# GAP-LAB-CUHK-SZ/RfDNet

Hardware: AMD Instinct MI355X
Metric: scenes/sec end-to-end reconstruction (ScanNet, 64^3 MISE) (higher is better)
Workload: dtype f32 (point ops, MLPs); f16x3 split MFMA with f32 accumulate (decoder, fp32-class)

## Files before the change

include/rfd_occ.h:

```cpp
#ifndef RFD_OCC_H
#define RFD_OCC_H

#include <stddef.h>

#ifdef __cplusplus
extern "C" {
#endif

#define RFD_OCC_HIDDEN 256
#define RFD_OCC_BLOCKS 5
#define RFD_OCC_TILE 128
#define RFD_OCC_TABLE_ROWS 23

#define RFD_OCC_MODE_F16X3 3
#define RFD_OCC_MODE_F16X1 1

size_t rfd_occ_packed_bytes(void);

int rfd_occ_pack_weights(const float *fc0_w, const float *fc1_w,
                         const int *kw0, int kw1, void *packed, void *stream);

int rfd_occ_decode(int n_tiles, const float *pts, const int *tile_prop,
                   const int *tile_src, const void *packed, const float *fc_p_w, const float *table,
                   const float *fc_out_w, float fc_out_b, float *logits,
                   int mode, void *stream);

int rfd_make_grid_points(int n, float lo, float hi, float scale, float *pts,
                         int n_padded, void *stream);

size_t rfd_mise_vstate_elems(int res0, int depth);
int rfd_mise_init(int K, int res0, int depth, unsigned char *pstate,
                  unsigned char *vstate, void *stream);
int rfd_mise_count(int K, int res0, int depth, const unsigned char *pstate,
                   int *counts, void *stream);
int rfd_mise_collect(int K, int res0, int depth, const unsigned char *pstate,
                     const int *offsets, int *cursors, float box_size,
                     float *pts, int *lin, void *stream);
int rfd_mise_scatter(int n_tiles, int res0, int depth, const int *tile_prop,
                     const int *tile_src, const int *lin, const float *logits,
                     float *values, unsigned char *pstate, void *stream);
int rfd_mise_subdivide(int K, int res0, int depth, double threshold,
                       const float *values, unsigned char *pstate,
                       unsigned char *vstate, void *stream);
int rfd_mise_subdivide_active(int K, int res0, int depth, double threshold, const float *values,
                              unsigned char *pstate, unsigned char *vstate, const int *evaluated,
                              void *stream);
size_t rfd_mise_dirty_elems(int res0, int depth);
int rfd_mise_subdivide_dirty(int K, int res0, int depth, double threshold, const float *values,
                             unsigned char *pstate, unsigned char *vstate, const int *evaluated, long long n_slots,
                             const int *lin, const int *tile_prop, unsigned char *dirty_cur,
                             unsigned char *dirty_next, int use_dirty, void *stream);
int rfd_mise_to_dense(int K, int res0, int depth, float *values,
                      unsigned char *pstate, void *stream);

int rfd_mc_blocks(int n);
int rfd_mc_classify(int K, int n, float pad_value, double iso, const float *grids,
                    unsigned char *code, int *vsum, int *tsum, void *stream);
int rfd_mc_emit_affine(int K, int n, float pad_value, double iso, const float *grids,
                       const unsigned char *code, const int *vblock, const int *tblock,
                       int *vbase, double *verts, int *tris, double va, double vc, void *stream);

int rfd_points_in_boxes(int b, int K, int n, int point_stride, const float *pts,
                        const double *boxes, int *counts, void *stream);
int rfd_nms3d(int b, int K, double iou_thr, int old_type, int use_cls, const double *aabb,
              const int *order, const int *cls, const unsigned char *valid,
              unsigned char *keep, void *stream);

int rfd_occ_pack_weights_w8(const float *fc0_w, const float *fc1_w, const int *kw0, int kw1,
                            void *packed, void *stream);
int rfd_occ_decode_w8(int n_tiles, const float *pts, const int *tile_prop, const int *tile_src,
                      const void *packed, const float *fc_p_w, const float *table,
                      const float *fc_out_w, float fc_out_b, float *logits, int mode, void *stream);
int rfd_occ_decode_scatter_w8(int n_tiles, const float *pts, const int *tile_prop, const int *tile_src,
                              const void *packed, const float *fc_p_w, const float *table,
                              const float *fc_out_w, float fc_out_b, const int *lin, float *values,
                              unsigned char *pstate, long long n_per, int mode, void *stream);

int rfd_occ_chunk_range(int k, int n_tiles, int n_workgroups, int *begin, int *end);
int rfd_occ_set_launch_shape(int static_partition, int cus, int chunk_cap);
int rfd_occ_set_tail_tiles(int n_tiles);
int rfd_occ_chunk_range_capped(int k, int n_tiles, int n_workgroups, int max_chunk, int *begin, int *end,
                               int *n_chunks);

int rfd_occ_normals_w8(int n_groups, const double *verts, const int *vend, const int *gprefix, int K,
                       const void *packed_fwd, const void *packed_bwd, const int *kw, const float *fc_p_w,
                       const float *table, const float *fc_out_w, float *normals, float *grad, int mode,
                       void *stream);

int rfd_refine_sample(int F, int K, const float *verts, const int *faces, const int *fend, const int *vend,
                      const int *tprefix, const float *eps, double *qd, float *qt, void *stream);
int rfd_refine_face_backward(int F, int K, const float *verts, const int *faces, const int *fend, const int *vend,
                             const int *tprefix, const float *eps, const float *logits, const float *grad, float tau,
                             double *cg, void *stream);
int rfd_refine_vertex_step(int V, const int *rowptr, const int *col, int n_corners, const double *cg, float *verts,
                           float *sq, float *gout, void *stream);
int rfd_refine_dirichlet(int n, unsigned long long seed, int step, float *out, void *stream);

size_t rfd_gemm_packed_bytes(int N, int K);
int rfd_gemm_pack_w(int N, int K, int sw, const float *W, void *packed, void *stream);
int rfd_gemm_f16x3(int M, int N, int K, const float *A, int lda, const void *packed_w,
                   float *C, int ldc, const float *bias, const float *gbias,
                   int rows_per_group, const float *R, int ldr, int relu_in, int relu_out,
                   int sa, int sw, float *pool_max, int pool_signed, void *stream);

// ... 37 lines not shown
```

rfdnet_amd/_lib.py:

```python
import ctypes as C
import os

_HERE = os.path.dirname(os.path.abspath(__file__))
LIB_PATH = os.environ.get("RFD_HIP_LIB") or os.path.join(_HERE, "lib", "librfd_hip.so")

_f = C.c_void_p
_i = C.c_int
_fl = C.c_float
_sz = C.c_size_t
_d = C.c_double

OPTIONAL = "optional"
ABI = {
    "furthest_point_sampling_kernel_wrapper": (_i, [_i, _i, _i, _f, _f, _f, _f]),
    "gather_points_kernel_wrapper": (_i, [_i, _i, _i, _i, _f, _f, _f, _f]),
    "gather_points_grad_kernel_wrapper": (_i, [_i, _i, _i, _i, _f, _f, _f, _f]),
    "query_ball_point_kernel_wrapper": (_i, [_i, _i, _i, _fl, _i, _f, _f, _f, _f]),
    "group_points_kernel_wrapper": (_i, [_i, _i, _i, _i, _i, _f, _f, _f, _f]),
    "group_points_grad_kernel_wrapper": (_i, [_i, _i, _i, _i, _i, _f, _f, _f, _f]),
    "three_nn_kernel_wrapper": (_i, [_i, _i, _i, _f, _f, _f, _f, _f]),
    "three_interpolate_kernel_wrapper": (_i, [_i, _i, _i, _i, _f, _f, _f, _f, _f]),
    "three_interpolate_grad_kernel_wrapper": (_i, [_i, _i, _i, _i, _f, _f, _f, _f, _f]),
    "rfd_group_concat": (_i, [_i, _i, _i, _i, _i, _fl, _i, _i, _f, _f, _f, _f, _f, _f, _f]),
    "rfd_furthest_point_sampling_gather": (_i, [_i, _i, _i, _f, _f, _f, _f, _f]),
    "rfd_chamfer_forward": (_i, [_i, _i, _f, _i, _f, _f, _f, _f, _f, _f]),
    "rfd_chamfer_backward": (_i, [_i, _i, _f, _i, _f, _f, _f, _f, _f, _f, _f, _f]),
    "rfd_sa_fused": (_i, [_i, _i, _i, _i, _i, _fl, _i, _f, _f, _f, _f, _i, _i, _i, _f, _f, _f, _f, _f, _f, _f, _f]),
    "rfd_occ_pack_weights": (_i, [_f, _f, C.POINTER(C.c_int), _i, _f, _f]),
    "rfd_occ_decode": (_i, [_i, _f, _f, _f, _f, _f, _f, _f, _fl, _f, _i, _f]),
    "rfd_occ_pack_weights_w8": (_i, [_f, _f, C.POINTER(C.c_int), _i, _f, _f]),
    "rfd_occ_decode_w8": (_i, [_i, _f, _f, _f, _f, _f, _f, _f, _fl, _f, _i, _f]),
    "rfd_occ_decode_scatter_w8": (_i, [_i, _f, _f, _f, _f, _f, _f, _f, _fl, _f, _f, _f, C.c_longlong, _i, _f]),
    "rfd_occ_chunk_range": (_i, [_i, _i, _i, C.POINTER(C.c_int), C.POINTER(C.c_int)]),
    "rfd_occ_chunk_range_capped": (_i, [_i, _i, _i, _i, C.POINTER(C.c_int), C.POINTER(C.c_int), C.POINTER(C.c_int)]),
    "rfd_occ_set_launch_shape": (_i, [_i, _i, _i]),
    "rfd_occ_set_tail_tiles": (_i, [_i]),
    "rfd_occ_normals_w8": (_i, [_i, _f, _f, _f, _i, _f, _f, C.POINTER(C.c_int), _f, _f, _f, _f, _f, _i, _f]),
    "rfd_refine_sample": (_i, [_i, _i, _f, _f, _f, _f, _f, _f, _f, _f, _f]),
    "rfd_refine_face_backward": (_i, [_i, _i, _f, _f, _f, _f, _f, _f, _f, _f, _fl, _f, _f]),
    "rfd_refine_vertex_step": (_i, [_i, _f, _f, _i, _f, _f, _f, _f, _f]),
    "rfd_refine_dirichlet": (_i, [_i, C.c_ulonglong, _i, _f, _f]),
    "rfd_fps_set_timeout_ms": (_i, [_i]),
    "rfd_fps_set_geometry": (_i, [_i]),
    "rfd_test_hold_cus": (_i, [_i, _f, _i, _f], OPTIONAL),
    "rfd_fps_test_phantom_units": (_i, [_i], OPTIONAL),
    "rfd_make_grid_points": (_i, [_i, _fl, _fl, _fl, _f, _i, _f]),
    "rfd_mise_init": (_i, [_i, _i, _i, _f, _f, _f]),
    "rfd_mise_count": (_i, [_i, _i, _i, _f, _f, _f]),
    "rfd_mise_collect": (_i, [_i, _i, _i, _f, _f, _f, _fl, _f, _f, _f]),
    "rfd_mise_scatter": (_i, [_i, _i, _i, _f, _f, _f, _f, _f, _f, _f]),
    "rfd_mise_subdivide": (_i, [_i, _i, _i, C.c_double, _f, _f, _f, _f]),
    "rfd_mise_subdivide_active": (_i, [_i, _i, _i, C.c_double, _f, _f, _f, _f, _f]),
    "rfd_mise_subdivide_dirty": (_i, [_i, _i, _i, C.c_double, _f, _f, _f, _f, C.c_longlong, _f, _f, _f, _f, _i, _f]),
    "rfd_mise_to_dense": (_i, [_i, _i, _i, _f, _f, _f]),
    "rfd_points_in_boxes": (_i, [_i, _i, _i, _i, _f, _f, _f, _f]),
    "rfd_nms3d": (_i, [_i, _i, C.c_double, _i, _i, _f, _f, _f, _f, _f, _f]),
    "rfd_gemm_pack_w": (_i, [_i, _i, _i, _f, _f, _f]),
    "rfd_gemm_f16x3": (_i, [_i, _i, _i, _f, _i, _f, _f, _i, _f, _f, _i, _f, _i, _i, _i, _i, _i, _f, _i, _f]),
    "rfd_mc_classify": (_i, [_i, _i, _fl, C.c_double, _f, _f, _f, _f, _f]),
    "rfd_mc_emit_affine": (_i, [_i, _i, _fl, C.c_double, _f, _f, _f, _f, _f, _f, _f, C.c_double, C.c_double, _f]),
    "rfd_mc_blocks": (_i, [_i]),
    "rfd_occ_fold_rows": (_i, [_i, _i, _i, _f, _f, _f, _f, _f, _f, _f, _i, _f, _f]),
    "rfd_rows3_rotate_z": (_i, [_i, _i, _f, _f, _f, _f]),
    "rfd_rows3_affine": (_i, [_i, _i, _f, _f, _f, _f]),
    "rfd_mlp_cols": (_i, [_i, _i, _i, _f, _f, _f, _f, _f, _f, _f]),
    "rfd_three_interpolate_cat": (_i, [_i, _i, _i, _i, _i, _f, _f, _f, _f, _f, _f]),
    "rfd_chain_pack_n": (_i, [_i, _i, _f, _f, _f, _i, _i, _i, _f, _f]),
    "rfd_chain_pool_n": (_i, [_i, _i, _i, _i, _i, _f, _i, _f, _f, _f, _f, _f, _i, _i, _i, _i, _i, _f, _f]),
    "rfd_head_pack": (_i, [_f, _f, _f, _i, _i, _i, _f, _f]),
    "rfd_head_scores": (_i, [_i, _i, _f, _i, _f, _f, _f, _f, _f, _f, _i, _i, _i, _i, _i, _f, _f]),
    "rfd_pos_embed": (_i, [_i, _i, _i, _f, _i, _f, _f, _i, _f, _f, _i, _f, _i, _i, _f]),
    "rfd_pos_embed_frag": (_i, [_i, _i, _i, _f, _i, _f, _f, _i, _f, _f, _i, _f, C.c_long, _i, _f]),
    "rfd_rows_to_frag": (_i, [_i, _i, _f, _i, _i, _i, _f, C.c_long, _f]),
    "rfd_frag_to_rows": (_i, [_i, _i, _f, C.c_long, _i, _f, _i, _f]),
    "rfd_gemm_f16x3_frag": (_i, [_i, _i, _i, _f, C.c_long, _f, _f, C.c_long, _f, _f, _i, _i, _i, _i, _f, _i, _f]),
    "rfd_box3d_iou": (_i, [_i, _i, _i, _f, _f, _f, _f, _f]),
    "rfd_ap_match": (_i, [_i, _i, _i, _i, _i, _f, _f, _f, _f, _f, _f, _f, _f]),
    "rfd_latent_prep": (_i, [_i, _i, _f, _f, _f, _f, _f, _f]),
    "rfd_latent_stage": (_i, [_i, _i, _i, _f, _f, _f, _f, _f, _f, _f, _f, _f]),
    "rfd_latent_head": (_i, [_i, _i, _f, _f, _f, _f, _f, _f, _f, _f, _f]),
    "rfd_bce_logits_rowsum": (_i, [_i, _i, _f, _i, _f, _i, _f, _f]),
    "rfd_voxel_iou": (_i, [_i, _i, _f, _i, _fl, _f, _f, _f, _f]),
    "rfd_vote_loss_partial": (_i, [_i, _i, _i, _i, _f, _f, _f, _f, _f, _f, _f]),
    "rfd_proposal_loss_partial": (_i, [_i, _i, _i, _i, _i, _i, _f, _f, _f, _f, _f, _f, _f, _f, C.POINTER(C.c_int), _f, _i, _f, _f,
                                       _f, _f, _f, _f, _f, _f, _f, _f, _i, _f, _f]),
    "rfd_detection_loss_finish": (_i, [_i, _i, _i, _f, _f, _f]),
    "rfd_mask_loss_partial": (_i, [_i, _i, _f, _f, _i, _f, _f, _f, _f]),
    "rfd_mask_loss_finish": (_i, [_i, _i, _fl, _f, _f, _f]),
    "rfd_fit_pose_run": (_i, [_i, _i, _i, _i, _i, _i, C.c_double, C.c_double, _f, _f, _f, _f, _f, _f, _f, _f, _f, _f, _f, _f,
                              _f, _f]),
    "rfd_raster_project": (_i, [_i, _i, _i, _f, _f, C.POINTER(C.c_double), C.c_double, _f, _f, _f, _f]),
    "rfd_raster_triangles": (_i, [_i, _i, _i, _i, _i, _i, _f, _f, _f, _f, _f, _f]),
    "rfd_raster_shade": (_i, [_i, _i, _i, _i, _i, _f, _f, _f, _f, _f, C.POINTER(C.c_double), _f, _f, _f, _f, _f]),
    "rfd_decimate_vertex_keys": (_i, [_i, _i, _i, _i, _f, _f, _f, _f, _f, _f]),
    "rfd_decimate_face_remap": (_i, [_i, _i, _i, _f, _f, _f, _f, _f, _f, _f, _f, _f]),
    "rfd_decimate_parity": (_i, [_i, _i, _i, _f, _f, _f, _f, _f, _f, _f]),
    "rfd_decimate_cell_solve": (_i, [_i, _i, _i, _i, _i, _f, _f, _f, _f, _f, _f, _f, _f, _f, C.c_double, _f, _f]),
    "rfd_decimate_compact_faces": (_i, [_i, _i, _f, _f, _f, _f, _f, _f, _f, _f]),
    "rfd_simplify_init": (_i, [_i, _i, _i, _i, _f, _f, _f, _f, _f, _f, _f, _f, _f]),
    "rfd_simplify_quadrics": (_i, [_i, _i, _f, _f, _f, _f, _f, _f]),
    "rfd_simplify_edges": (_i, [_i, _i, _f, _f, _f, _f, _f, _f, _f, _f, _f, _f]),
    "rfd_simplify_edge_costs": (_i, [_i, _i, _i, _f, _f, _f, _f, _f, _f, _f, _f, _f, _f, _f, _f, _f, _f, _f, _f]),
    "rfd_simplify_vertex_min": (_i, [_i, _i, _i, _f, _f, _f, _f, _f, _f, _f]),
    "rfd_simplify_select": (_i, [_i, _i, _f, _f, _f, _f, _f, _f, _f]),
    "rfd_simplify_apply": (_i, [_i, _i, _f, _f, _f, _f, _f, _f, _f, _f, _f, _f, _f]),
    "rfd_simplify_compact_faces": (_i, [_i, _i, _i, _f, _f, _f, _f, _f, _f, _f, _f, _f, _f, _f]),
# ... 247 lines not shown
```

rfdnet_amd/csrc/mise.hip:

```cpp
#include "common.h"
#include "../../include/rfd_occ.h"

namespace {

__host__ __device__ inline size_t cube(size_t n) { return n * n * n; }

__host__ __device__ inline size_t vstate_offset(int res0, int l) {
  size_t o = 0;
  for (int i = 0; i < l; ++i) o += cube((size_t)res0 << i);
  return o;
}

__global__ void grid_points_kernel(int n, float lo, float hi, float scale,
                                   float *__restrict__ pts, int n_padded) {
  const int e = blockIdx.x * blockDim.x + threadIdx.x;
  if (e >= n_padded) return;
  const int total = n * n * n;
  float x = 0.f, y = 0.f, z = 0.f;
  if (e < total) {
    const int k = e % n, j = (e / n) % n, i = e / (n * n);
    const float step = n > 1 ? (hi - lo) / (float)(n - 1) : 0.f;
    const int half = n / 2;
    auto ax = [&](int q) { return q < half ? lo + step * (float)q : hi - step * (float)(n - 1 - q); };
    x = scale * ax(i);
// ... 111 lines not shown
__global__ __launch_bounds__(256) void mise_collect_kernel(
    int R1, size_t total, size_t n_per, int K, const unsigned char *__restrict__ pstate,
    const int *__restrict__ offsets, int *__restrict__ cursors, float box_size,
    float *__restrict__ pts, int *__restrict__ lin) {
  const size_t chunk = (size_t)blockIdx.x * blockDim.x + threadIdx.x;
  const int lane = threadIdx.x & 63;
  unsigned m = 0, lo = 0xffffu;
  int k0 = -1;
  size_t e0 = 0;
  if (chunk * 16 < total) {
    const Chunk c = load_chunk(pstate, total, n_per, chunk);
    m = unknown_mask16(c);
    lo = c.split >= 16 ? 0xffffu : ((1u << c.split) - 1u);
    k0 = c.k0;
    e0 = c.e0;
  }
  const int c0 = __popc(m & lo), c1 = __popc(m & ~lo);
  if (!__any(c0 | c1)) return;
  int base0 = 0, base1 = 0;
  const int kf = __shfl(k0, 0);
  if (__all((k0 == kf || (c0 | c1) == 0) && c1 == 0)) {
    int incl = c0;
#pragma unroll
    for (int off = 1; off < 64; off <<= 1) {
      const int o = __shfl_up(incl, off);
      if (lane >= off) incl += o;
    }
    const int tot = __shfl(incl, 63);
    int wb = 0;
    if (lane == 0) wb = atomicAdd(cursors + kf, tot);
    wb = __shfl(wb, 0);
    base0 = wb + incl - c0;
  } else {
    if (c0) base0 = atomicAdd(cursors + k0, c0);
    if (c1 && k0 + 1 < K) base1 = atomicAdd(cursors + k0 + 1, c1);
  }
  const float res = (float)(R1 - 1);
  unsigned mm = m;
  while (mm) {
    const int j = __ffs(mm) - 1;
    mm &= mm - 1;
    const bool second = !((lo >> j) & 1u);
    const int k = second ? k0 + 1 : k0;
    if (k >= K) break;
    const unsigned e = (unsigned)(second ? (e0 + j - n_per) : (e0 + j));
    const int slot = offsets[k] + (second ? base1++ : base0++);
    const unsigned row = e / (unsigned)R1;
    const int kz = (int)(e - row * (unsigned)R1), ix = (int)(row / (unsigned)R1),
              jy = (int)(row - (unsigned)ix * (unsigned)R1);
    pts[(size_t)slot * 3 + 0] = box_size * ((float)ix / res - 0.5f);
    pts[(size_t)slot * 3 + 1] = box_size * ((float)jy / res - 0.5f);
    pts[(size_t)slot * 3 + 2] = box_size * ((float)kz / res - 0.5f);
    lin[slot] = (int)e;
  }
}

__global__ void mise_scatter_kernel(size_t n_per, const int *__restrict__ tile_prop,
                                    const int *__restrict__ tile_src,
                                    const int *__restrict__ lin,
                                    const float *__restrict__ logits,
                                    float *__restrict__ values,
                                    unsigned char *__restrict__ pstate) {
  const int tile = blockIdx.x;
  const int k = tile_prop[tile];
  if (k < 0) return;
  const size_t slot = (size_t)tile * RFD_OCC_TILE + threadIdx.x;
  const int l = lin[tile_src ? (size_t)tile_src[tile] * RFD_OCC_TILE + threadIdx.x : slot];
  if (l < 0) return;
  values[(size_t)k * n_per + l] = logits[slot];
  pstate[(size_t)k * n_per + l] = 2;
}

constexpr int SUB_TJ = 8, SUB_TK = 32;

__host__ __device__ inline int sub_tiles_k(int nl) { return (nl + SUB_TK - 1) / SUB_TK; }
__host__ __device__ inline int sub_tiles_j(int nl) { return (nl + SUB_TJ - 1) / SUB_TJ; }
__host__ __device__ inline size_t dirty_offset(int res0, int l) {
  size_t o = 0;
  for (int i = 0; i < l; ++i) {
    const int nl = res0 << i;
    o += (size_t)sub_tiles_k(nl) * sub_tiles_j(nl) * nl;
  }
  return o;
}
__device__ inline size_t dirty_tile(int nl, int vi, int vj, int vk) {
  return ((size_t)vi * sub_tiles_j(nl) + vj / SUB_TJ) * sub_tiles_k(nl) + vk / SUB_TK;
}
__device__ inline void mark_children(unsigned char *dirty_next, int res0, int l, int nl, int vi, int vj, int vk) {
  unsigned char *d = dirty_next + dirty_offset(res0, l + 1);
  d[dirty_tile(2 * nl, 2 * vi, 2 * vj, 2 * vk)] = 1;
  d[dirty_tile(2 * nl, 2 * vi + 1, 2 * vj, 2 * vk)] = 1;
}

__global__ void mise_mark_dirty_kernel(size_t n_slots, int R1, int res0, int depth, const int *__restrict__ lin,
                                       const int *__restrict__ tile_prop, size_t d_per,
                                       unsigned char *__restrict__ dirty) {
  const size_t i = (size_t)blockIdx.x * blockDim.x + threadIdx.x;
  if (i >= n_slots) return;
  const int p = lin[i];
  if (p < 0) return;
  const int kp = tile_prop[i / RFD_OCC_TILE];
  if (kp < 0) return;
  const int c[3] = {p / (R1 * R1), (p / R1) % R1, p % R1};
  unsigned char *dk = dirty + (size_t)kp * d_per;
  for (int l = 0; l < depth; ++l) {
    const int s = 1 << (depth - l), nl = res0 << l;
// ... 114 lines not shown
#pragma unroll
      for (int i = 0; i < 16; ++i) {
        const int rel = rel0 + i;
        if (rel < 0 || rel >= plane) continue;
        unsigned char f = 0;
        if (rel < run && ((w[i >> 2] >> (8 * (i & 3))) & 0xffu) == 2u) {
          const double v = (double)vals[base + rel];
          f = 4 | (v >= thr ? 1 : 0) | (v <= thr ? 2 : 0);
        }
        flags[a * plane + rel] = f;
      }
    }
  } else {
    for (int t = threadIdx.x; t < (s + 1) * PJ * PK; t += SUB_TJ * SUB_TK) {
      const int c = t % PK, b = (t / PK) % PJ, a = t / (PK * PJ);
      unsigned char f = 0;
      if (y0 + b < R1 && z0 + c < R1) {
        const size_t p = ((size_t)(x0 + a) * R1 + (y0 + b)) * R1 + (z0 + c);
        if (ps[p] == 2) {
          const double v = (double)vals[p];
          f = 4 | (v >= thr ? 1 : 0) | (v <= thr ? 2 : 0);
        }
      }
      flags[t] = f;
    }
  }
  __syncthreads();
  if (!leaf) return;
  unsigned any = 0;
  for (int a = 0; a <= s; ++a)
    for (int b = 0; b <= s; ++b)
      for (int c = 0; c <= s; ++c)
        any |= flags[(a * PJ + tj * s + b) * PK + tk * s + c];
  if ((any & 3) != 3) return;
  vs[e] = 2;
  if (l + 1 < depth) {
    unsigned char *vc = vstate + (size_t)kp * v_per + vstate_offset(res0, l + 1);
    const int nc = nl * 2;
    for (int a = 0; a < 2; ++a)
      for (int b = 0; b < 2; ++b)
        for (int c = 0; c < 2; ++c)
          vc[((size_t)(2 * vi + a) * nc + (2 * vj + b)) * nc + (2 * vk + c)] = 1;
    if (dirty_next) mark_children(dirty_next + (size_t)kp * d_per, res0, l, nl, vi, vj, vk);
  }
  const int h = s >> 1;
  for (int a = 0; a < 3; ++a)
    for (int b = 0; b < 3; ++b)
      for (int c = 0; c < 3; ++c) {
        const size_t p = ((size_t)(x0 + a * h) * R1 + (y0 + tj * s + b * h)) * R1 + (z0 + tk * s + c * h);
        if (ps[p] == 0) ps[p] = 1;
      }
}

__global__ void mise_fill_kernel(int R1, int axis, size_t n_per, float *__restrict__ values,
                                 unsigned char *__restrict__ pstate) {
  const int line = blockIdx.x * blockDim.x + threadIdx.x;
  if (line >= R1 * R1) return;
  const int kp = blockIdx.y;
  const int u = line / R1, v = line % R1;
  size_t stride, start;
  if (axis == 0) { stride = (size_t)R1 * R1; start = (size_t)u * R1 + v; }
  else if (axis == 1) { stride = R1; start = (size_t)u * R1 * R1 + v; }
  else { stride = 1; start = ((size_t)u * R1 + v) * R1; }
  float *vals = values + (size_t)kp * n_per;
  unsigned char *ps = pstate + (size_t)kp * n_per;
  bool prev_valid = false;
  float prev = 0.f;
  for (int q0 = 0; q0 < R1; q0 += 8) {
    float v[8];
    unsigned char st[8];
#pragma unroll
    for (int u = 0; u < 8; ++u) {
      const bool in = q0 + u < R1;
      const size_t p = start + (size_t)(q0 + u) * stride;
      st[u] = in ? ps[p] : 0;
      v[u] = in ? vals[p] : 0.f;
    }
#pragma unroll
    for (int u = 0; u < 8; ++u) {
      if (q0 + u >= R1) break;
      const size_t p = start + (size_t)(q0 + u) * stride;
      const bool valid = st[u] >= 2;
      if (!valid && prev_valid) {
        vals[p] = prev;
        ps[p] = 3;
      }
      prev = valid ? v[u] : prev;
      prev_valid = valid || prev_valid;
    }
  }
}

__global__ __launch_bounds__(256) void mise_fill_yz_kernel(int R1, size_t n_per,
                                                           float *__restrict__ values,
                                                           const unsigned char *__restrict__ pstate) {
  extern __shared__ float plane_v[];
  const int n2 = R1 * R1;
  unsigned char *plane_s = reinterpret_cast<unsigned char *>(plane_v + n2);
  const size_t base = (size_t)blockIdx.y * n_per + (size_t)blockIdx.x * n2;
  for (int t = threadIdx.x; t < n2; t += 256) {
    plane_v[t] = values[base + t];
    plane_s[t] = pstate[base + t];
  }
  __syncthreads();
  for (int axis = 1; axis <= 2; ++axis) {
    if ((int)threadIdx.x < R1) {
// ... 59 lines not shown
  RFD_CHECK_LAUNCH();
  return 0;
}

RFD_API size_t rfd_mise_vstate_elems(int res0, int depth) {
  const size_t v = vstate_offset(res0, depth);
  return v ? v : 1;
}

RFD_API int rfd_mise_init(int K, int res0, int depth, unsigned char *pstate,
                          unsigned char *vstate, void *stream) {
  if (K <= 0) return 0;
  const int R1 = (res0 << depth) + 1;
  const size_t n_per = cube((size_t)R1);
  hipStream_t s = (hipStream_t)stream;
  RFD_CHECK(hipMemsetAsync(pstate, 0, n_per * (size_t)K, s));
  const int L = res0 + 1;
  hipLaunchKernelGGL(mise_init_points_kernel, dim3((unsigned)((L * L * L + 255) / 256), K), dim3(256),
                     0, s, R1, 1 << depth, L, n_per, pstate);
  RFD_CHECK_LAUNCH();
  const size_t v_per = rfd_mise_vstate_elems(res0, depth);
  hipLaunchKernelGGL(mise_init_voxels_kernel, dim3((unsigned)((v_per + 255) / 256), K), dim3(256),
                     0, s, depth > 0 ? cube((size_t)res0) : 0, v_per, vstate);
  RFD_CHECK_LAUNCH();
  return 0;
}

RFD_API int rfd_mise_count(int K, int res0, int depth, const unsigned char *pstate,
                           int *counts, void *stream) {
  if (K <= 0) return 0;
  const int R1 = (res0 << depth) + 1;
  const size_t n_per = cube((size_t)R1);
  hipStream_t s = (hipStream_t)stream;
  RFD_CHECK(hipMemsetAsync(counts, 0, sizeof(int) * K, s));
  hipLaunchKernelGGL(mise_count_kernel, dim3(COUNT_PARTS, K), dim3(256), 0, s, n_per, pstate, counts);
  RFD_CHECK_LAUNCH();
  return 0;
}

RFD_API int rfd_mise_collect(int K, int res0, int depth, const unsigned char *pstate,
                             const int *offsets, int *cursors, float box_size,
                             float *pts, int *lin, void *stream) {
  if (K <= 0) return 0;
  const int R1 = (res0 << depth) + 1;
  const size_t n_per = cube((size_t)R1);
  const size_t total = n_per * (size_t)K, chunks = (total + 15) / 16;
  hipLaunchKernelGGL(mise_collect_kernel, dim3((unsigned)((chunks + 255) / 256)), dim3(256), 0,
                     (hipStream_t)stream, R1, total, n_per, K, pstate, offsets, cursors, box_size,
                     pts, lin);
  RFD_CHECK_LAUNCH();
  return 0;
}

RFD_API int rfd_mise_scatter(int n_tiles, int res0, int depth, const int *tile_prop,
                             const int *tile_src, const int *lin, const float *logits,
                             float *values, unsigned char *pstate, void *stream) {
  if (n_tiles <= 0) return 0;
  const int R1 = (res0 << depth) + 1;
  hipLaunchKernelGGL(mise_scatter_kernel, dim3(n_tiles), dim3(RFD_OCC_TILE), 0,
                     (hipStream_t)stream, cube((size_t)R1), tile_prop, tile_src, lin, logits, values,
                     pstate);
  RFD_CHECK_LAUNCH();
  return 0;
}

static int mise_subdivide(int K, int res0, int depth, double threshold, const float *values,
                          unsigned char *pstate, unsigned char *vstate, const int *evaluated, void *stream,
                          const unsigned char *dirty_cur = nullptr, unsigned char *dirty_next = nullptr) {
  if (K <= 0 || depth <= 0) return 0;
  const int R1 = (res0 << depth) + 1;
  const size_t n_per = cube((size_t)R1);
  const size_t v_per = rfd_mise_vstate_elems(res0, depth);
  const size_t d_per = dirty_offset(res0, depth);
  for (int l = depth - 1; l >= 0; --l) {
    const size_t nvox = cube((size_t)res0 << l);
    const int sl = 1 << (depth - l), nl = res0 << l;
    if (sl <= 4) {
      const unsigned tiles = (unsigned)(ceil_div(nl, SUB_TK) * ceil_div(nl, SUB_TJ) * nl);
      const size_t lds = (size_t)(sl + 1) * (SUB_TJ * sl + 1) * (SUB_TK * sl + 1);
      hipLaunchKernelGGL(mise_subdivide_lds_kernel, dim3(tiles, K), dim3(SUB_TJ * SUB_TK), lds,
                         (hipStream_t)stream, R1, res0, depth, l, threshold, n_per, v_per,
                         n_per * (size_t)K, values, pstate, vstate, evaluated, d_per, dirty_cur, dirty_next);
      RFD_CHECK_LAUNCH();
      continue;
    }
    hipLaunchKernelGGL(mise_subdivide_kernel, dim3((unsigned)((nvox + 255) / 256), K), dim3(256), 0,
                       (hipStream_t)stream, R1, res0, depth, l, threshold, n_per, v_per, values,
                       pstate, vstate, evaluated, d_per, dirty_next);
    RFD_CHECK_LAUNCH();
  }
  return 0;
}

RFD_API int rfd_mise_subdivide(int K, int res0, int depth, double threshold,
                               const float *values, unsigned char *pstate,
                               unsigned char *vstate, void *stream) {
  return mise_subdivide(K, res0, depth, threshold, values, pstate, vstate, nullptr, stream);
}

RFD_API int rfd_mise_subdivide_active(int K, int res0, int depth, double threshold,
                                      const float *values, unsigned char *pstate,
                                      unsigned char *vstate, const int *evaluated, void *stream) {
  return mise_subdivide(K, res0, depth, threshold, values, pstate, vstate, evaluated, stream);
}

RFD_API size_t rfd_mise_dirty_elems(int res0, int depth) { return dirty_offset(res0, depth); }

RFD_API int rfd_mise_subdivide_dirty(int K, int res0, int depth, double threshold, const float *values,
                                     unsigned char *pstate, unsigned char *vstate, const int *evaluated,
                                     long long n_slots, const int *lin, const int *tile_prop, unsigned char *dirty_cur,
                                     unsigned char *dirty_next, int use_dirty, void *stream) {
  if (K <= 0 || depth <= 0) return 0;
  if (!dirty_cur || !dirty_next || (use_dirty && (!lin || !tile_prop || n_slots < 0))) {
    return rfd_invalid("rfd_mise_subdivide_dirty: dirty maps / query list");
  }
  const int R1 = (res0 << depth) + 1;
  const size_t d_per = dirty_offset(res0, depth);
  if (use_dirty && n_slots > 0) {
    hipLaunchKernelGGL(mise_mark_dirty_kernel, dim3((unsigned)((n_slots + 255) / 256)), dim3(256), 0, (hipStream_t)stream,
                       (size_t)n_slots, R1, res0, depth, lin, tile_prop, d_per, dirty_cur);
    RFD_CHECK_LAUNCH();
  }
  const int rc = mise_subdivide(K, res0, depth, threshold, values, pstate, vstate, evaluated, stream,
                                use_dirty ? dirty_cur : nullptr, dirty_next);
  if (rc) return rc;
  RFD_CHECK(hipMemsetAsync(dirty_cur, 0, (size_t)K * d_per, (hipStream_t)stream));
  return 0;
}

RFD_API int rfd_mise_to_dense(int K, int res0, int depth, float *values,
                              unsigned char *pstate, void *stream) {
  if (K <= 0) return 0;
  const int R1 = (res0 << depth) + 1;
  const size_t n_per = cube((size_t)R1);
  const size_t plane_lds = (size_t)R1 * R1 * 5;
  const bool fused = plane_lds <= 64 * 1024 && R1 <= 256;
  for (int axis = 0; axis < (fused ? 1 : 2); ++axis) {
    hipLaunchKernelGGL(mise_fill_kernel, dim3(ceil_div(R1 * R1, 256), K), dim3(256), 0,
                       (hipStream_t)stream, R1, axis, n_per, values, pstate);
    RFD_CHECK_LAUNCH();
  }
  if (fused)
    hipLaunchKernelGGL(mise_fill_yz_kernel, dim3(R1, K), dim3(256), plane_lds, (hipStream_t)stream,
                       R1, n_per, values, pstate);
  else
    hipLaunchKernelGGL(mise_fill_z_kernel, dim3(ceil_div(R1 * R1, 4), K), dim3(256), 0,
                       (hipStream_t)stream, R1, n_per, values, pstate);
  RFD_CHECK_LAUNCH();
  return 0;
}
```

rfdnet_amd/iscnet/generator.py:

```python
import os

import numpy as np
import torch

from .. import _lib, mesh_batch, ragged
from .occ_decoder import GROUP, MODE_F16X3, TILE, logit_threshold, run_with_range_fallback


class Mesh(object):

    def __init__(self, vertices, faces, vertex_normals=None):
        self.vertices = vertices
        self.faces = faces
        self.vertex_normals = vertex_normals


def draw_dirichlet(face_counts, steps):
    total = int(sum(face_counts))
    out = np.empty((steps, total, 3), dtype=np.float32)
    at = 0
    for n in face_counts:
        for it in range(steps):
            if n:
                out[it, at:at + n] = np.random.dirichlet((0.5, 0.5, 0.5), size=n)
# ... 62 lines not shown
        return self.extract_meshes(grids, fold=fold[0] if self._needs_fold() else None)

    def generate_from_latent(self, z, c=None, device='cuda', **kwargs):
        fold = []
        grids = self._grids(z, c, fold_out=fold)
        return self.extract_meshes(grids, fold=fold[0] if self._needs_fold() else None)[0]

    def eval_points(self, p, z, c=None, device='cuda', **kwargs):
        with torch.no_grad():
            return self.model.decode(p.unsqueeze(0).to(c.device), z, c, **kwargs).logits.squeeze(0)

    def logit_threshold(self):
        return logit_threshold(self.threshold)

    def generate_grids(self, object_features, cls_codes=None, fold_out=None):
        self.model.eval()
        if getattr(self.model, 'use_cls_for_completion', False):
            object_features = torch.cat([object_features, cls_codes], dim=-1)
        K = object_features.size(0)
        z = self.model.get_z_from_prior((K,), sample=self.sample, device=object_features.device)
        return self._grids(z, object_features, fold_out=fold_out)

    @torch.no_grad()
    def _grids(self, z, c, fold_out=None):
        dec = self.model.decoder
        dev = c.device
        K = c.size(0)
        box_size = 1 + self.padding
        table, fc_p_w = dec.fold(z.float(), c.float())
        if fold_out is not None:
            fold_out.append((table, fc_p_w))
        if self.upsampling_steps == 0:
            nx = self.resolution0
            total = nx ** 3
            tiles_per = int(ragged.blocks(total, TILE))
            pts = torch.empty(tiles_per * TILE, 3, dtype=torch.float32, device=dev)
            _lib.call("rfd_make_grid_points", dev, nx, -0.5, 0.5, float(box_size), pts.data_ptr(),
                      tiles_per * TILE)
            tile_prop, tile_src = ragged.uniform_maps(K, tiles_per, dev)
            logits = dec.decode_tiles(pts, tile_prop, table, fc_p_w, tile_src=tile_src)
            self.stats = {'n_queries': K * total, 'rounds': 1, 'per_round': [K * total]}
            return logits.view(K, tiles_per * TILE)[:, :total].reshape(K, nx, nx, nx)
        return self._grids_mise(dec, table, fc_p_w, K, dev, box_size)

    def _grids_mise(self, dec, table, fc_p_w, K, dev, box_size):
        res0, depth = self.resolution0, self.upsampling_steps
        R1 = (res0 << depth) + 1
        n_per = R1 ** 3
        lib = _lib.lib()
        v_per = lib.rfd_mise_vstate_elems(res0, depth)
        values = torch.empty(K, n_per, dtype=torch.float32, device=dev)
        pstate = torch.empty(K, n_per, dtype=torch.uint8, device=dev)
        vstate = torch.empty(K, v_per, dtype=torch.uint8, device=dev)
        counts = torch.empty(K, dtype=torch.int32, device=dev)
        dirty = torch.zeros(2, K, lib.rfd_mise_dirty_elems(res0, depth), dtype=torch.uint8, device=dev)
        _lib.call("rfd_mise_init", dev, K, res0, depth, pstate.data_ptr(), vstate.data_ptr())
        thr = self.logit_threshold()
        n_queries, rounds = 0, 0
        per_round = []
        while True:
            shared = rounds == 0 and self._round0(res0, depth, box_size, K, dev)
            if shared:
                pts, lin, tile_prop, tile_src, total = shared
                n_tiles = tile_prop.numel()
            else:
                _lib.call("rfd_mise_count", dev, K, res0, depth, pstate.data_ptr(), counts.data_ptr())
                cnt = counts.cpu().numpy().astype(np.int64)
                total = int(cnt.sum())
                if total == 0:
                    break
                tiles = ragged.padded_tiles(cnt, TILE)
                n_tiles = int(tiles.prefix[-1])
                tile_prop = ragged.to_int32(tiles.owner, dev)
                tile_src = None
                offsets = ragged.to_int32(tiles.slot[:-1], dev)
                cursors = torch.zeros(K, dtype=torch.int32, device=dev)
                pts = torch.zeros(n_tiles * TILE, 3, dtype=torch.float32, device=dev)
                lin = torch.full((n_tiles * TILE,), -1, dtype=torch.int32, device=dev)
                _lib.call("rfd_mise_collect", dev, K, res0, depth, pstate.data_ptr(), offsets.data_ptr(),
                          cursors.data_ptr(), float(box_size), pts.data_ptr(), lin.data_ptr())
            if self.round_hook is not None:
                self.round_hook(rounds, depth)
            if dec.can_scatter():
                dec.decode_tiles(pts, tile_prop, table, fc_p_w, tile_src=tile_src, scatter=(lin, values, pstate))
            else:
                logits = dec.decode_tiles(pts, tile_prop, table, fc_p_w, tile_src=tile_src)
                _lib.call("rfd_mise_scatter", dev, n_tiles, res0, depth, tile_prop.data_ptr(),
                          _lib.ptr(tile_src), lin.data_ptr(), logits.data_ptr(), values.data_ptr(), pstate.data_ptr())
            sparse = (not shared) and total <= K * self.sparse_round_points
            _lib.call("rfd_mise_subdivide_dirty", dev, K, res0, depth, float(thr), values.data_ptr(),
                      pstate.data_ptr(), vstate.data_ptr(), None if shared else counts.data_ptr(),
                      int(lin.numel()) if sparse else 0, lin.data_ptr() if sparse else None,
                      tile_prop.data_ptr() if sparse else None, dirty[rounds & 1].data_ptr(),
                      dirty[(rounds + 1) & 1].data_ptr(), int(sparse))
            n_queries += total
            per_round.append(total)
            rounds += 1
        _lib.call("rfd_mise_to_dense", dev, K, res0, depth, values.data_ptr(), pstate.data_ptr())
        self.stats = {'n_queries': n_queries, 'rounds': rounds, 'per_round': per_round}
        return values.view(K, R1, R1, R1)

    def _round0(self, res0, depth, box_size, K, dev):
        def build():
            R1 = (res0 << depth) + 1
            ps = torch.empty(1, R1 ** 3, dtype=torch.uint8, device=dev)
            vs = torch.empty(1, _lib.lib().rfd_mise_vstate_elems(res0, depth), dtype=torch.uint8, device=dev)
            cnt = torch.empty(1, dtype=torch.int32, device=dev)
            _lib.call("rfd_mise_init", dev, 1, res0, depth, ps.data_ptr(), vs.data_ptr())
            _lib.call("rfd_mise_count", dev, 1, res0, depth, ps.data_ptr(), cnt.data_ptr())
            n = int(cnt.item())
            tiles_per = int(ragged.blocks(n, TILE))
            pts = torch.zeros(tiles_per * TILE, 3, dtype=torch.float32, device=dev)
            lin = torch.full((tiles_per * TILE,), -1, dtype=torch.int32, device=dev)
            offsets = torch.zeros(1, dtype=torch.int32, device=dev)
            cursors = torch.zeros(1, dtype=torch.int32, device=dev)
            _lib.call("rfd_mise_collect", dev, 1, res0, depth, ps.data_ptr(), offsets.data_ptr(),
                      cursors.data_ptr(), float(box_size), pts.data_ptr(), lin.data_ptr())
            return (pts, lin) + ragged.uniform_maps(K, tiles_per, dev) + (K * n,)
        return self._round0_cache.get((res0, depth, float(box_size), K, str(dev)), build, dev)

    def extract_meshes(self, grids, fold=None):
        from .mcubes import marching_cubes_batch
        thr = self.logit_threshold()
        n = grids.shape[1]
        box_size = 1 + self.padding
        a = box_size / (n - 1)
        v, f, vend, tend = marching_cubes_batch(grids, thr, pad_value=-1e6, return_flat=True,
                                                affine=(a, -1.5 * a - 0.5 * box_size))
        if self.decimate_cells:
            from .decimate import decimate_meshes
            K = len(vend) - 1
            v, f, vend, tend = decimate_meshes(v, f, vend, tend, self.decimate_cells, lo=np.full((K, 3), -box_size / 2),
                                               h=np.full(K, box_size / self.decimate_cells))
        if self.simplify_faces:
            from .simplify import simplify_meshes
            v, f, vend, tend, _ = simplify_meshes(v, f, vend, tend, self.simplify_faces)
        self.last_normals = None
        refine = self.refinement_step > 0
        if refine and fold is None:
            raise ValueError("refinement needs fold = (table, fc_p_w) of the meshes' codes (DecoderCBatchNorm.fold)")
        nrm = None
        if fold is not None and (self.with_normals or not refine):
            nrm = self.last_normals = self.model.decoder.normals(v if v.dtype == torch.float64 else v.double(), vend,
                                                                 fold[0], fold[1])
        if refine:
            v = self.refine_meshes(v, f, vend, tend, fold, self.refinement_step)
        self.last_buffers = (v, f, vend, tend)
# ... 104 lines not shown
```

Baseline: 20.10.

## Fuse MISE round-0 subdivide with counting and pad-aware wave-level collect

Adds a dedicated round-0 subdivide kernel that evaluates the coarse lattice in LDS tiles, marks split voxels and children, and accumulates per-proposal point counts in one pass, so round 1 skips the separate count kernel. Replaces the collect kernel with a wave-compacting version that uses block-level cursor reservation when a block covers one proposal and writes tile padding itself, which removes the zero/fill initialisation of pts and lin. Dirty buffers and counts now share one zeroed allocation. The round-0 path relies on counts being zero at entry and falls back to the generic path when LDS needs exceed 64 KB.

```diff
diff --git a/include/rfd_occ.h b/include/rfd_occ.h
--- a/include/rfd_occ.h
+++ b/include/rfd_occ.h
@@ -50,6 +50,12 @@
                              unsigned char *pstate, unsigned char *vstate, const int *evaluated, long long n_slots,
                              const int *lin, const int *tile_prop, unsigned char *dirty_cur,
                              unsigned char *dirty_next, int use_dirty, void *stream);
+int rfd_mise_subdivide_round0(int K, int res0, int depth, double threshold, const float *values,
+                              unsigned char *pstate, unsigned char *vstate, unsigned char *dirty_next,
+                              int *counts, void *stream);
+int rfd_mise_collect_padded(int K, int res0, int depth, const unsigned char *pstate, const int *counts,
+                            const int *offsets, int *cursors, float box_size, int pad_to, float *pts, int *lin,
+                            void *stream);
 int rfd_mise_to_dense(int K, int res0, int depth, float *values,
                       unsigned char *pstate, void *stream);
 
diff --git a/rfdnet_amd/_lib.py b/rfdnet_amd/_lib.py
--- a/rfdnet_amd/_lib.py
+++ b/rfdnet_amd/_lib.py
@@ -52,6 +52,8 @@
     "rfd_mise_subdivide": (_i, [_i, _i, _i, C.c_double, _f, _f, _f, _f]),
     "rfd_mise_subdivide_active": (_i, [_i, _i, _i, C.c_double, _f, _f, _f, _f, _f]),
     "rfd_mise_subdivide_dirty": (_i, [_i, _i, _i, C.c_double, _f, _f, _f, _f, C.c_longlong, _f, _f, _f, _f, _i, _f]),
+    "rfd_mise_subdivide_round0": (_i, [_i, _i, _i, C.c_double, _f, _f, _f, _f, _f, _f]),
+    "rfd_mise_collect_padded": (_i, [_i, _i, _i, _f, _f, _f, _f, _fl, _i, _f, _f, _f]),
     "rfd_mise_to_dense": (_i, [_i, _i, _i, _f, _f, _f]),
     "rfd_points_in_boxes": (_i, [_i, _i, _i, _i, _f, _f, _f, _f]),
     "rfd_nms3d": (_i, [_i, _i, C.c_double, _i, _i, _f, _f, _f, _f, _f, _f]),
diff --git a/rfdnet_amd/csrc/mise.hip b/rfdnet_amd/csrc/mise.hip
--- a/rfdnet_amd/csrc/mise.hip
+++ b/rfdnet_amd/csrc/mise.hip
@@ -187,6 +187,131 @@
     pts[(size_t)slot * 3 + 1] = box_size * ((float)jy / res - 0.5f);
     pts[(size_t)slot * 3 + 2] = box_size * ((float)kz / res - 0.5f);
     lin[slot] = (int)e;
+  }
+}
+
+constexpr int COL_SEG = 4;
+
+__device__ __forceinline__ unsigned unknown_mask16(const uint4 v) {
+  Chunk c;
+  c.w[0] = v.x; c.w[1] = v.y; c.w[2] = v.z; c.w[3] = v.w;
+  return unknown_mask16(c);
+}
+
+__global__ __launch_bounds__(256) void mise_collect_wave_kernel(
+    int R1, size_t total, size_t n_per, int K, const unsigned char *__restrict__ pstate,
+    const int *__restrict__ counts, const int *__restrict__ offsets, int *__restrict__ cursors, float box_size,
+    int pad_to, float *__restrict__ pts, int *__restrict__ lin) {
+  __shared__ unsigned short rel[4][1024];
+  __shared__ int unit_base[4 * COL_SEG];
+  const int lane = threadIdx.x & 63, wave = threadIdx.x >> 6;
+  const size_t wave_b0 = ((size_t)blockIdx.x * 4 + wave) * (size_t)(COL_SEG * 1024);
+  uint4 v[COL_SEG];
+#pragma unroll
+  for (int q = 0; q < COL_SEG; ++q) {
+    const size_t b0 = wave_b0 + (size_t)q * 1024 + (size_t)lane * 16;
+    v[q] = make_uint4(0u, 0u, 0u, 0u);
+    if (b0 + 16 <= total) {
+      v[q] = *reinterpret_cast<const uint4 *>(pstate + b0);
+    } else if (b0 < total) {
+      unsigned w[4] = {0u, 0u, 0u, 0u};
+      for (int j = 0; j < 16; ++j)
+        if (b0 + j < total) w[j >> 2] |= (unsigned)pstate[b0 + j] << (8 * (j & 3));
+      v[q] = make_uint4(w[0], w[1], w[2], w[3]);
+    }
+  }
+  const size_t blk_b0 = (size_t)blockIdx.x * 4 * (size_t)(COL_SEG * 1024);
+  const size_t blk_b1 = blk_b0 + 4 * (size_t)(COL_SEG * 1024) < total ? blk_b0 + 4 * (size_t)(COL_SEG * 1024) : total;
+  const bool single = blk_b0 < total && blk_b0 / n_per == (blk_b1 - 1) / n_per;
+  if (single) {
+#pragma unroll
+    for (int q = 0; q < COL_SEG; ++q) {
+      const int t = wave_sum(__popc(unknown_mask16(v[q])));
+      if (lane == 0) unit_base[wave * COL_SEG + q] = t;
+    }
+    __syncthreads();
+    if (threadIdx.x == 0) {
+      int run = 0;
+      for (int u = 0; u < 4 * COL_SEG; ++u) {
+        const int t = unit_base[u];
+        unit_base[u] = run;
+        run += t;
+      }
+      const int first = run ? atomicAdd(cursors + (int)(blk_b0 / n_per), run) : 0;
+      for (int u = 0; u < 4 * COL_SEG; ++u) unit_base[u] += first;
+    }
+    __syncthreads();
+  }
+  const float res = (float)(R1 - 1);
+#pragma unroll
+  for (int q = 0; q < COL_SEG; ++q) {
+    const unsigned m = unknown_mask16(v[q]);
+    if (!__syncthreads_or((int)m)) continue;
+    const int c = __popc(m);
+    int incl = c;
+#pragma unroll
+    for (int off = 1; off < 64; off <<= 1) {
+      const int o = __shfl_up(incl, off);
+      if (lane >= off) incl += o;
+    }
+    const int T = __shfl(incl, 63);
+    {
+      unsigned mm = m;
+      int pos = incl - c;
+      while (mm) {
+        rel[wave][pos++] = (unsigned short)(lane * 16 + __ffs(mm) - 1);
+        mm &= mm - 1;
+      }
+    }
+    __syncthreads();
+    const size_t seg_b0 = wave_b0 + (size_t)q * 1024;
+    const int k0 = (int)(seg_b0 / n_per);
+    const size_t e0 = seg_b0 - (size_t)k0 * n_per;
+    for (int base = 0; base < T; base += 64) {
+      const int i = base + lane;
+      const bool active = i < T;
+      int k = -1;
+      unsigned e = 0;
+      if (active) {
+        size_t ee = e0 + rel[wave][i];
+        k = k0;
+        while (ee >= n_per) { ee -= n_per; ++k; }
+        e = (unsigned)ee;
+      }
+      const int prevk = __shfl_up(k, 1);
+      const bool head = active && (lane == 0 || k != prevk);
+      const unsigned long long hb = __ballot(head), ab = __ballot(active);
+      const unsigned long long upto = lane == 63 ? ~0ull : ((2ull << lane) - 1ull);
+      const unsigned long long below = hb & upto, above = hb & ~upto;
+      const int hl = below ? 63 - __clzll((long long)below) : 0;
+      const int end = above ? __ffsll((long long)above) - 1 : __popcll(ab);
+      int wb = 0;
+      if (!single && head && k < K) wb = atomicAdd(cursors + k, end - lane);
+      wb = __shfl(wb, hl);
+      if (active && k < K) {
+        const int slot = offsets[k] + (single ? unit_base[wave * COL_SEG + q] + i : wb + (lane - hl));
+        const unsigned row = e / (unsigned)R1;
+        const int kz = (int)(e - row * (unsigned)R1), ix = (int)(row / (unsigned)R1),
+                  jy = (int)(row - (unsigned)ix * (unsigned)R1);
+        pts[(size_t)slot * 3 + 0] = box_size * ((float)ix / res - 0.5f);
+        pts[(size_t)slot * 3 + 1] = box_size * ((float)jy / res - 0.5f);
+        pts[(size_t)slot * 3 + 2] = box_size * ((float)kz / res - 0.5f);
+        lin[slot] = (int)e;
+      }
+    }
+    __syncthreads();
+  }
+  const size_t kq = (size_t)blockIdx.x * 4 + wave;
+  if (kq < (size_t)K) {
+    const int cnt = counts[kq];
+    const int end = (cnt + pad_to - 1) / pad_to * pad_to;
+    for (int i = cnt + lane; i < end; i += 64) {
+      const size_t slot = (size_t)offsets[kq] + i;
+      pts[slot * 3 + 0] = 0.f;
+      pts[slot * 3 + 1] = 0.f;
+      pts[slot * 3 + 2] = 0.f;
+      lin[slot] = -1;
+    }
   }
 }
 
@@ -407,6 +532,101 @@
       }
 }
 
+constexpr int R0_TI = 4;
+
+__host__ __device__ inline size_t round0_lds(int res0) {
+  const size_t L = (size_t)res0 + 1;
+  return (R0_TI + 2) * L * L + (R0_TI + 1) * (size_t)res0 * res0;
+}
+
+__global__ __launch_bounds__(256) void mise_round0_kernel(
+    int R1, int res0, int depth, double thr, size_t n_per, size_t v_per, const float *__restrict__ values,
+    unsigned char *__restrict__ pstate, unsigned char *__restrict__ vstate, size_t d_per,
+    unsigned char *__restrict__ dirty_next, int *__restrict__ counts) {
+  extern __shared__ unsigned char r0_lds[];
+  __shared__ int wsum[4];
+  const int L = res0 + 1, nl = res0, s = 1 << depth, h = s >> 1;
+  unsigned char *lat = r0_lds;
+  unsigned char *spl = r0_lds + (size_t)(R0_TI + 2) * L * L;
+  const int i0 = blockIdx.x * R0_TI, kp = blockIdx.y;
+  const int ni = L - i0 < R0_TI ? L - i0 : R0_TI;
+  const float *vals = values + (size_t)kp * n_per;
+  unsigned char *ps = pstate + (size_t)kp * n_per;
+  const int n_lat = (ni + 2) * L * L;
+#pragma unroll 4
+  for (int t = threadIdx.x; t < n_lat; t += 256) {
+    const int a = t / (L * L), r = t - a * L * L, j = r / L, k = r - j * L;
+    const int li = i0 - 1 + a;
+    unsigned char f = 0;
+    if (li >= 0 && li < L) {
+      const double v = (double)vals[((size_t)(li * s) * R1 + (size_t)(j * s)) * R1 + (size_t)(k * s)];
+      f = (v >= thr ? 1 : 0) | (v <= thr ? 2 : 0);
+    }
+    lat[t] = f;
+  }
+  __syncthreads();
+  const int n_vox = (ni + 1) * nl * nl;
+  for (int t = threadIdx.x; t < n_vox; t += 256) {
+    const int b = t / (nl * nl), r = t - b * nl * nl, vj = r / nl, vk = r - vj * nl;
+    const int vi = i0 - 1 + b;
+    unsigned char sp = 0;
+    if (vi >= 0 && vi < nl) {
+      unsigned any = 0;
+#pragma unroll
+      for (int c = 0; c < 8; ++c) any |= lat[((b + (c >> 2)) * L + vj + ((c >> 1) & 1)) * L + vk + (c & 1)];
+      sp = (any & 3) == 3;
+      if (sp && b > 0) {
+        vstate[(size_t)kp * v_per + ((size_t)vi * nl + vj) * nl + vk] = 2;
+        if (depth > 1) {
+          unsigned char *vc = vstate + (size_t)kp * v_per + vstate_offset(res0, 1);
+          const int nc = nl * 2;
+          for (int a = 0; a < 2; ++a)
+            for (int bb = 0; bb < 2; ++bb)
+              for (int c = 0; c < 2; ++c)
+                vc[((size_t)(2 * vi + a) * nc + (2 * vj + bb)) * nc + (2 * vk + c)] = 1;
+          if (dirty_next) mark_children(dirty_next + (size_t)kp * d_per, res0, 0, nl, vi, vj, vk);
+        }
+      }
+    }
+    spl[t] = sp;
+  }
+  __syncthreads();
+  int cnt = 0;
+  const int n_node = ni * L * L;
+  for (int t = threadIdx.x; t < n_node; t += 256) {
+    const int a = t / (L * L), r = t - a * L * L, j = r / L, k = r - j * L;
+    const int i = i0 + a;
+    unsigned sm = 0;
+#pragma unroll
+    for (int d = 0; d < 8; ++d) {
+      const int dx = d >> 2, dy = (d >> 1) & 1, dz = d & 1;
+      const int vi = i - dx, vj = j - dy, vk = k - dz;
+      if (vi >= 0 && vi < nl && vj >= 0 && vj < nl && vk >= 0 && vk < nl && spl[((a + 1 - dx) * nl + vj) * nl + vk])
+        sm |= 1u << d;
+    }
+    if (!sm) continue;
+#pragma unroll
+    for (int o = 1; o < 8; ++o) {
+      const int oa = o >> 2, ob = (o >> 1) & 1, oc = o & 1;
+      unsigned allow = 0;
+#pragma unroll
+      for (int d = 0; d < 8; ++d)
+        if (!((d >> 2) & oa) && !(((d >> 1) & 1) & ob) && !((d & 1) & oc)) allow |= 1u << d;
+      if (sm & allow) {
+        ps[((size_t)(i * s + oa * h) * R1 + (size_t)(j * s + ob * h)) * R1 + (size_t)(k * s + oc * h)] = 1;
+        ++cnt;
+      }
+    }
+  }
+  cnt = wave_sum(cnt);
+  if ((threadIdx.x & 63) == 0) wsum[threadIdx.x >> 6] = cnt;
+  __syncthreads();
+  if (threadIdx.x == 0) {
+    const int tot = wsum[0] + wsum[1] + wsum[2] + wsum[3];
+    if (tot) atomicAdd(counts + kp, tot);
+  }
+}
+
 __global__ void mise_fill_kernel(int R1, int axis, size_t n_per, float *__restrict__ values,
                                  unsigned char *__restrict__ pstate) {
   const int line = blockIdx.x * blockDim.x + threadIdx.x;
@@ -572,6 +792,22 @@
   return 0;
 }
 
+RFD_API int rfd_mise_collect_padded(int K, int res0, int depth, const unsigned char *pstate, const int *counts,
+                                    const int *offsets, int *cursors, float box_size, int pad_to, float *pts, int *lin,
+                                    void *stream) {
+  if (K <= 0) return 0;
+  if (pad_to <= 0 || !counts) return rfd_invalid("rfd_mise_collect_padded: counts / pad_to");
+  const int R1 = (res0 << depth) + 1;
+  const size_t n_per = cube((size_t)R1);
+  const size_t total = n_per * (size_t)K, per_block = (size_t)4 * COL_SEG * 1024;
+  size_t blocks = (total + per_block - 1) / per_block;
+  if (blocks < (size_t)(K + 3) / 4) blocks = (size_t)(K + 3) / 4;
+  hipLaunchKernelGGL(mise_collect_wave_kernel, dim3((unsigned)blocks), dim3(256), 0, (hipStream_t)stream, R1, total,
+                     n_per, K, pstate, counts, offsets, cursors, box_size, pad_to, pts, lin);
+  RFD_CHECK_LAUNCH();
+  return 0;
+}
+
 RFD_API int rfd_mise_scatter(int n_tiles, int res0, int depth, const int *tile_prop,
                              const int *tile_src, const int *lin, const float *logits,
                              float *values, unsigned char *pstate, void *stream) {
@@ -648,6 +884,28 @@
   return 0;
 }
 
+RFD_API int rfd_mise_subdivide_round0(int K, int res0, int depth, double threshold, const float *values,
+                                      unsigned char *pstate, unsigned char *vstate, unsigned char *dirty_next,
+                                      int *counts, void *stream) {
+  if (K <= 0 || depth <= 0) return 0;
+  if (!counts) return rfd_invalid("rfd_mise_subdivide_round0: counts");
+  const int R1 = (res0 << depth) + 1;
+  const size_t n_per = cube((size_t)R1);
+  const size_t lds = round0_lds(res0);
+  if (lds > 64 * 1024) {
+    const int rc = mise_subdivide(K, res0, depth, threshold, values, pstate, vstate, nullptr, stream, nullptr, dirty_next);
+    if (rc) return rc;
+    hipLaunchKernelGGL(mise_count_kernel, dim3(COUNT_PARTS, K), dim3(256), 0, (hipStream_t)stream, n_per, pstate, counts);
+    RFD_CHECK_LAUNCH();
+    return 0;
+  }
+  hipLaunchKernelGGL(mise_round0_kernel, dim3((unsigned)ceil_div(res0 + 1, R0_TI), K), dim3(256), lds, (hipStream_t)stream,
+                     R1, res0, depth, threshold, n_per, rfd_mise_vstate_elems(res0, depth), values, pstate, vstate,
+                     dirty_offset(res0, depth), dirty_next, counts);
+  RFD_CHECK_LAUNCH();
+  return 0;
+}
+
 RFD_API int rfd_mise_to_dense(int K, int res0, int depth, float *values,
                               unsigned char *pstate, void *stream) {
   if (K <= 0) return 0;
diff --git a/rfdnet_amd/iscnet/generator.py b/rfdnet_amd/iscnet/generator.py
--- a/rfdnet_amd/iscnet/generator.py
+++ b/rfdnet_amd/iscnet/generator.py
@@ -138,8 +138,11 @@
         values = torch.empty(K, n_per, dtype=torch.float32, device=dev)
         pstate = torch.empty(K, n_per, dtype=torch.uint8, device=dev)
         vstate = torch.empty(K, v_per, dtype=torch.uint8, device=dev)
-        counts = torch.empty(K, dtype=torch.int32, device=dev)
-        dirty = torch.zeros(2, K, lib.rfd_mise_dirty_elems(res0, depth), dtype=torch.uint8, device=dev)
+        d_per = lib.rfd_mise_dirty_elems(res0, depth)
+        c_off = (2 * K * d_per + 3) // 4 * 4
+        zeroed = torch.zeros(c_off + 4 * K, dtype=torch.uint8, device=dev)
+        dirty = zeroed[:2 * K * d_per].view(2, K, d_per)
+        counts = zeroed[c_off:].view(torch.int32)
         _lib.call("rfd_mise_init", dev, K, res0, depth, pstate.data_ptr(), vstate.data_ptr())
         thr = self.logit_threshold()
         n_queries, rounds = 0, 0
@@ -150,7 +153,8 @@
                 pts, lin, tile_prop, tile_src, total = shared
                 n_tiles = tile_prop.numel()
             else:
-                _lib.call("rfd_mise_count", dev, K, res0, depth, pstate.data_ptr(), counts.data_ptr())
+                if rounds != 1:
+                    _lib.call("rfd_mise_count", dev, K, res0, depth, pstate.data_ptr(), counts.data_ptr())
                 cnt = counts.cpu().numpy().astype(np.int64)
                 total = int(cnt.sum())
                 if total == 0:
@@ -161,10 +165,10 @@
                 tile_src = None
                 offsets = ragged.to_int32(tiles.slot[:-1], dev)
                 cursors = torch.zeros(K, dtype=torch.int32, device=dev)
-                pts = torch.zeros(n_tiles * TILE, 3, dtype=torch.float32, device=dev)
-                lin = torch.full((n_tiles * TILE,), -1, dtype=torch.int32, device=dev)
-                _lib.call("rfd_mise_collect", dev, K, res0, depth, pstate.data_ptr(), offsets.data_ptr(),
-                          cursors.data_ptr(), float(box_size), pts.data_ptr(), lin.data_ptr())
+                pts = torch.empty(n_tiles * TILE, 3, dtype=torch.float32, device=dev)
+                lin = torch.empty(n_tiles * TILE, dtype=torch.int32, device=dev)
+                _lib.call("rfd_mise_collect_padded", dev, K, res0, depth, pstate.data_ptr(), counts.data_ptr(),
+                          offsets.data_ptr(), cursors.data_ptr(), float(box_size), TILE, pts.data_ptr(), lin.data_ptr())
             if self.round_hook is not None:
                 self.round_hook(rounds, depth)
             if dec.can_scatter():
@@ -174,11 +178,15 @@
                 _lib.call("rfd_mise_scatter", dev, n_tiles, res0, depth, tile_prop.data_ptr(),
                           _lib.ptr(tile_src), lin.data_ptr(), logits.data_ptr(), values.data_ptr(), pstate.data_ptr())
             sparse = (not shared) and total <= K * self.sparse_round_points
-            _lib.call("rfd_mise_subdivide_dirty", dev, K, res0, depth, float(thr), values.data_ptr(),
-                      pstate.data_ptr(), vstate.data_ptr(), None if shared else counts.data_ptr(),
-                      int(lin.numel()) if sparse else 0, lin.data_ptr() if sparse else None,
-                      tile_prop.data_ptr() if sparse else None, dirty[rounds & 1].data_ptr(),
-                      dirty[(rounds + 1) & 1].data_ptr(), int(sparse))
+            if shared:
+                _lib.call("rfd_mise_subdivide_round0", dev, K, res0, depth, float(thr), values.data_ptr(),
+                          pstate.data_ptr(), vstate.data_ptr(), dirty[1].data_ptr(), counts.data_ptr())
+            else:
+                _lib.call("rfd_mise_subdivide_dirty", dev, K, res0, depth, float(thr), values.data_ptr(),
+                          pstate.data_ptr(), vstate.data_ptr(), counts.data_ptr(),
+                          int(lin.numel()) if sparse else 0, lin.data_ptr() if sparse else None,
+                          tile_prop.data_ptr() if sparse else None, dirty[rounds & 1].data_ptr(),
+                          dirty[(rounds + 1) & 1].data_ptr(), int(sparse))
             n_queries += total
             per_round.append(total)
             rounds += 1
```

Result: no change. 20.07, median of 3 (-0.1%).
